# DeepMotionAIResearch/DenseMatchingBenchmark

Hardware: AMD Instinct MI355X
Metric: stereo pairs/s (540x960, max_disp=192) (higher is better)
Workload: dtype f32; 1 GPU; PSMNet Concatenation-volume + 3D aggregation + soft-argmin, 544x960 (540x960 padded), max_disp=192, batch 4 per GPU; costs_materialised=True, conv3d_mode=exact

## Files before the change

densematchingbenchmark_amd/csrc/catconv.hip:

```cpp
#include "dmb_common.h"

namespace dmb {

typedef float f32x4_t __attribute__((ext_vector_type(4)));

__global__ __launch_bounds__(256) void copy_window_kernel(const float* __restrict__ src, float* __restrict__ dst,
                                                          long long rows, int W, int Wd, int xs) {
  const long long total = rows * Wd;
  for (long long i = blockIdx.x * 256LL + threadIdx.x; i < total; i += (long long)gridDim.x * 256) {
    const long long r = i / Wd;
    const int j = (int)(i - r * Wd), g = j + xs;
    dst[i] = (g >= 0 && g < W) ? src[r * W + g] : 0.f;
  }
}

__global__ __launch_bounds__(256) void zero_columns_kernel(float* __restrict__ t, long long rows, int pitch, int x0) {
  const int n = pitch - x0;
  const long long total = rows * n;
  for (long long i = blockIdx.x * 256LL + threadIdx.x; i < total; i += (long long)gridDim.x * 256) {
    const long long r = i / n;
    t[r * pitch + x0 + (int)(i - r * n)] = 0.f;
  }
}

// ... 98 lines not shown
        f[e] = u >= 2 ? f[e] : (u >= -2 ? t : 0.f);
      }
    }
    const float g3 = border ? gbz : g[3];
    float4 o;
    o.x = fmaxf(fmaf(f[0] + g[0], sc, sh), lo);
    o.y = fmaxf(fmaf(f[1] + g[1], sc, sh), lo);
    o.z = fmaxf(fmaf(f[2] + g[2], sc, sh), lo);
    o.w = fmaxf(fmaf(f[3] + g3, sc, sh), lo);
    __builtin_nontemporal_store(f32x4_t{o.x, o.y, o.z, o.w}, reinterpret_cast<f32x4_t*>(op + (size_t)z * HW));
  };
  if (zlo == 0) {
    const float4 a1 = fa4(1), a2 = fa4(2);
    float g[4];
#pragma unroll
    for (int e = 0; e < 4; ++e) g[e] = hc1(1, x + e) + hc1(2, x + e - 1);
    plane(0, make_float4(a1.x + a2.x, a1.y + a2.y, a1.z + a2.z, a1.w + a2.w), g, band[0], gb[0]);
  }
  const float4 fm = *reinterpret_cast<const float4*>(FM + row * W + x);
  auto gml = [&](int n) { return gm_row[n > -4 ? n : -4]; };
  constexpr int ZB = 4;
  float win[ZB + 3], gbw[ZB];
  float4 bnd[ZB];
  auto load_block = [&](int z0, float (&w)[ZB + 3], float4 (&bq)[ZB], float (&gq)[ZB]) {
#pragma unroll
    for (int i = 0; i < ZB + 3; ++i) w[i] = gml(x - z0 + 3 - i);
#pragma unroll
    for (int k = 0; k < ZB; ++k) {
      const int z = z0 + k < D ? z0 + k : D - 1;
      if (NEAR) bq[k] = (x - z >= -5 && x - z <= 1) ? band[z] : make_float4(0.f, 0.f, 0.f, 0.f);
      if (!NEAR) gq[k] = gb[z];
    }
  };
  const int zb = zlo > 1 ? zlo : 1, ze = zhi < D - 1 ? zhi : D - 1;
  load_block(zb, win, bnd, gbw);
  for (int z0 = zb; z0 < ze; z0 += ZB) {
    float nwin[ZB + 3], ngbw[ZB];
    float4 nbnd[ZB];
    if (z0 + ZB < ze) load_block(z0 + ZB, nwin, nbnd, ngbw);
#pragma unroll
    for (int k = 0; k < ZB; ++k) {
      if (z0 + k < ze) {
        const float g[4] = {win[3 + k], win[2 + k], win[1 + k], win[k]};
        plane(z0 + k, fm, g, bnd[k], gbw[k]);
      }
    }
#pragma unroll
    for (int i = 0; i < ZB + 3; ++i) win[i] = nwin[i];
#pragma unroll
    for (int k = 0; k < ZB; ++k) {
      bnd[k] = nbnd[k];
      gbw[k] = ngbw[k];
    }
  }
  if (zhi == D) {
    const float4 a0 = fa4(0), a1 = fa4(1);
    const int u0 = x - (D - 1);
    float g[4];
#pragma unroll
    for (int e = 0; e < 4; ++e) g[e] = hc1(0, u0 + e + 1) + hc1(1, u0 + e);
    plane(D - 1, make_float4(a0.x + a1.x, a0.y + a1.y, a0.z + a1.z, a0.w + a1.w), g, band[D - 1], gb[D - 1]);
  }
}

template <bool NEAR>
__global__ __launch_bounds__(256) void catconv_combine_kernel(const float* __restrict__ FA, const float* __restrict__ HC,
                                                              const float* __restrict__ FM, const float* __restrict__ BAND,
                                                              const float* __restrict__ GM, const float* __restrict__ GB,
                                                              const float* __restrict__ scale, const float* __restrict__ shift,
                                                              float* __restrict__ out, long long rows, int Co, int CA, int D,
                                                              int H, int W, int XS, int relu) {
  constexpr int ZSPLIT = NEAR ? 4 : 1;
  const int W4 = NEAR ? XS >> 2 : (W - XS) >> 2;
  long long idx = blockIdx.x * 256LL + threadIdx.x;
  if (idx >= rows * W4 * ZSPLIT) return;
  const int zc = (int)(idx / (rows * W4));
  idx -= zc * (rows * W4);
  const long long rowid = idx / W4;
  const int dz = D / ZSPLIT;
  catconv_combine_body<NEAR>(FA, HC, FM, BAND, GM, GB, scale, shift, out, Co, CA, D, H, W, relu, rowid,
                             (int)(idx - rowid * W4) * 4 + (NEAR ? 0 : XS), zc * dz, (zc + 1) * dz);
}

}

using namespace dmb;

extern "C" int dmb_copy_window_f32(const float* src, float* dst, long long rows, int W, int Wd, int xs, void* stream) {
  if (!src || !dst || rows <= 0 || W <= 0 || Wd <= 0) return fail(DMB_EINVAL, "copy_window: bad argument");
  const long long total = rows * Wd;
  const int blocks = (int)((total + 255) / 256 < 65536 ? (total + 255) / 256 : 65536);
  hipLaunchKernelGGL(copy_window_kernel, dim3(blocks), dim3(256), 0, (hipStream_t)stream, src, dst, rows, W, Wd, xs);
  return launch_status("copy_window launch failed");
}

extern "C" int dmb_zero_columns_f32(float* t, long long rows, int pitch, int x0, void* stream) {
  if (!t || rows <= 0 || pitch <= 0 || x0 < 0 || x0 > pitch) return fail(DMB_EINVAL, "zero_columns: bad argument");
  if (x0 == pitch) return DMB_OK;
  const long long total = rows * (pitch - x0);
  const int blocks = (int)((total + 255) / 256 < 65536 ? (total + 255) / 256 : 65536);
  hipLaunchKernelGGL(zero_columns_kernel, dim3(blocks), dim3(256), 0, (hipStream_t)stream, t, rows, pitch, x0);
  return launch_status("zero_columns launch failed");
}

extern "C" int dmb_catconv_finalize_f32(const float* FA, const float* FB, const float* HC, const float* HD, float* FM,
                                        float* BAND, float* GM, float* GB, int B, int Co, int CA, int CB, int D, int H, int W,
                                        int Wc, void* stream) {
  if (!FA || !FB || !HC || !HD || !FM || !BAND || !GM || !GB || B <= 0 || Co <= 0 || D < 3 || H <= 0 || W <= 0 || (W & 3) ||
      CA < 3 * Co || CB < 6 * Co || (CB & 1) || Wc > W || Wc < D + 2 || (((uintptr_t)FA | (uintptr_t)FM) & 15))
    return fail(DMB_EINVAL, "catconv_finalize: bad argument");
  const long long rows = (long long)B * Co * H;
  if (rows > 0x7fffffffLL) return fail(DMB_EUNSUPPORTED, "catconv_finalize: grid too large");
  hipLaunchKernelGGL(catconv_finalize_kernel, dim3((unsigned)rows), dim3(256), 0, (hipStream_t)stream, FA, FB, HC, HD, FM, BAND,
                     GM, GB, B, Co, CA, CB, D, H, W, Wc);
  return launch_status("catconv_finalize launch failed");
}

extern "C" int dmb_catconv_combine_f32(const float* FA, const float* HC, const float* FM, const float* BAND, const float* GM,
                                       const float* GB, const float* scale, const float* shift, float* out, int B, int Co,
                                       int CA, int D, int H, int W, int relu, void* stream) {
  if (!FA || !HC || !FM || !BAND || !GM || !GB || !out || B <= 0 || Co <= 0 || CA < 3 * Co || D < 3 || (D & 3) || H <= 0 ||
      W <= 0 || (W & 3) || W < D + 8 || (((uintptr_t)FA | (uintptr_t)FM | (uintptr_t)BAND | (uintptr_t)out) & 15))
    return fail(DMB_EINVAL, "catconv_combine: bad argument (D, W multiples of 4, W >= D + 8, tensors 16-byte aligned)");
  int XS = (D + 4 + 15) / 16 * 16;
  if (XS > W - 4) XS = W - 4;
  const long long rows = (long long)B * Co * H, tn = rows * (XS / 4) * 4, tf = rows * ((W - XS) / 4);
  if ((tf + 255) / 256 > 0x7fffffffLL || (tn + 255) / 256 > 0x7fffffffLL) return fail(DMB_EUNSUPPORTED, "catconv_combine: grid too large");
  hipLaunchKernelGGL(catconv_combine_kernel<false>, dim3((unsigned)((tf + 255) / 256)), dim3(256), 0, (hipStream_t)stream, FA,
                     HC, FM, BAND, GM, GB, scale, shift, out, rows, Co, CA, D, H, W, XS, relu);
  hipLaunchKernelGGL(catconv_combine_kernel<true>, dim3((unsigned)((tn + 255) / 256)), dim3(256), 0, (hipStream_t)stream, FA,
                     HC, FM, BAND, GM, GB, scale, shift, out, rows, Co, CA, D, H, W, XS, relu);
  return launch_status("catconv_combine launch failed");
}
```

densematchingbenchmark_amd/ops.py:

```python
import ctypes

import torch

from . import _lib, param_state
from ._lib import check, dev_ptr, host_floats, host_ints, launch, opt, stream_ptr
from .param_state import bump_param_epoch, param_epoch


def disp_index_list(max_disp, start_disp=0, dilation=1):
    end_disp = start_disp + max_disp - 1
    n = (max_disp + dilation - 1) // dilation
    return [int(v) for v in torch.linspace(start_disp, end_disp, n)]


def disp_sample_values(max_disp, start_disp=0, dilation=1):
    end_disp = start_disp + max_disp - 1
    n = (max_disp + dilation - 1) // dilation
    return [float(v) for v in torch.linspace(start_disp, end_disp, n)]


class KernelTimer:

    def __init__(self, tags, every=1):
        self.tags = set(tags)
# ... 284 lines not shown
AUTO_OVERLAP_MAX_VOXELS = 48 * 136 * 240
_side_streams = {}


def set_branch_overlap(flag):
    global _branch_overlap
    _branch_overlap = "auto" if flag == "auto" else bool(flag)


def branch_overlap(raw_cost=None):
    if _branch_overlap != "auto":
        return _branch_overlap
    if raw_cost is None:
        return False
    B, _, D, H, W = raw_cost.shape
    return B * D * H * W <= AUTO_OVERLAP_MAX_VOXELS


def side_stream(device, which=0):
    key = (device.index if device.index is not None else torch.cuda.current_device(), which)
    if key not in _side_streams:
        _side_streams[key] = torch.cuda.Stream(device)
    return _side_streams[key]


_view_streams = True


def set_view_streams(flag):
    global _view_streams
    _view_streams = bool(flag)


def view_streams():
    return _view_streams


def warm_packed_parameters(module):
    stamp = param_state.module_stamp(module)
    if module.__dict__.get("_dmb_warmed") == stamp:
        return
    for m in module.modules():
        pre = getattr(m, "_prepacked", None)
        if pre is not None:
            pre()
    module.__dict__["_dmb_warmed"] = stamp


def _map_tensors(f, out):
    if torch.is_tensor(out):
        return f(out)
    return type(out)(_map_tensors(f, o) for o in out)


def two_view_forward(fn, left, right, module=None):
    if not (_view_streams and left.is_cuda):
        B = left.shape[0]
        f = fn(torch.cat((left, right), 0))
        return _map_tensors(lambda t: t[:B], f), _map_tensors(lambda t: t[B:], f)
    if module is not None:
        warm_packed_parameters(module)
    main = torch.cuda.current_stream(left.device)
    side = side_stream(left.device, 2)
    fork = main.record_event()
    with torch.cuda.stream(side):
        side.wait_event(fork)
        fr = fn(right)
        _map_tensors(lambda t: t.record_stream(main), fr)
        right.record_stream(side)
        done = side.record_event()
    fl = fn(left)
    main.wait_event(done)
    return fl, fr


_first_layer_mode = "merged"


def set_first_layer_mode(mode):
    global _first_layer_mode
    if mode not in ("merged", "streams", "serial"):
        raise ValueError("first-layer mode must be 'merged', 'streams' or 'serial'")
    _first_layer_mode = mode


def set_first_layer_streams(flag):
    set_first_layer_mode("streams" if flag else "serial")


def copy_window(src, Wd, xs):
    sh = _lib.shim()
    if sh is not None:
        return sh.copy_window(src if src.is_contiguous() else src.contiguous(), int(Wd), int(xs))
    src = _f32c(src, "src")
    W = src.shape[-1]
    dst = torch.empty(tuple(src.shape[:-1]) + (Wd,), dtype=torch.float32, device=src.device)
    launch("dmb_copy_window_f32", src, dst, src.numel() // W, W, Wd, xs)
    return dst


def zero_columns_(t, x0):
    if t.dtype != torch.float32 or not t.is_contiguous():
        raise _lib.DmbLibraryError("zero_columns_: contiguous float32 tensor expected")
    pitch = t.shape[-1]
    launch("dmb_zero_columns_f32", t, t.numel() // pitch, pitch, x0)
    return t


DECONV_PLAN_SPLIT_K, DECONV_PLAN_QUEUE, DECONV_PLAN_PARITY = 1, 2, 3
CONV_PLAN_SPLIT_K, CONV_PLAN_S1_VEC, CONV_PLAN_S1_FLAT, CONV_PLAN_S1_C128, CONV_PLAN_S2 = 1, 2, 3, 4, 5


def _align(t):
    p = 0 if t is None else t.data_ptr()
    return min(p & -p or 16, 16)


def conv3d_k3_plan(x, Co, stride=1, residual=None, out=None, ncu=0):
    shape = tuple(x) if isinstance(x, (tuple, list)) else tuple(x.shape)
    B, Ci, D, H, W = (int(v) for v in shape)
    xa = 16 if isinstance(x, (tuple, list)) else _align(x)
    stride = _hw_stride(stride, "conv3d_k3_plan")
    if stride == "hw":
        raise _lib.DmbLibraryError("conv3d_k3_plan: stride (1, 2, 2) is dmb_conv3d_k3_hw_f32's, which has one form")
    return _lib.load().dmb_conv3d_k3_plan(B, Ci, int(Co), D, H, W, int(stride), xa, _align(out), _align(residual), 0 if _split_k else 1, int(ncu))


def padded_rows_applicable(x, Co):
    B, Ci, D, H, W = x.shape
    if not (x.is_cuda and W % 4 == 2):
        return False
    plan = _lib.load().dmb_deconv3d_k3s2_plan(B, Ci, Co, D, H, (W + 3) // 4 * 4, 2 * W, min(x.data_ptr() & -x.data_ptr() or 16, 16), 16, 16, 16, 1, 0)
    return plan >> 8 == DECONV_PLAN_QUEUE


CATCONV_CH = 128


def catconv_applicable(L, R, disp_idx, Co):
    if not _cat_fusion or L.dim() != 4 or L.shape != R.shape:
        return False
    D, W = len(disp_idx), L.shape[3]
    return (list(disp_idx) == list(range(D)) and D >= 4 and D % 4 == 0 and W % 4 == 0 and W >= D + 8 and Co <= 32
            and L.dtype == torch.float32 and L.is_cuda)


def catconv_pack(w, kind="cat"):
    lib = _lib.load()
    w = _f32c(w.detach(), "weight")
    Co = w.shape[0]
    C = w.shape[1] if kind == "dif" else w.shape[1] // 2
    n = lib.dmb_conv2d_packed_floats(CATCONV_CH, C, 3)
    buf = torch.empty((5, n), dtype=torch.float32, device=w.device)
    launch("dmb_catconv_pack_weights_f32", w, buf, Co, C, CATCONV_CH, 1 if kind == "dif" else 0)
    return {"A": buf[0], "B1": buf[1], "B2": buf[2], "HC": buf[3], "HD": buf[4], "Co": Co, "Cin": C}


def catconv_pack_torch(w, kind="cat"):
    Co = w.shape[0]
    w = w.detach().float()
    if kind == "dif":
        wl, wr = w, -w
    else:
        C = w.shape[1] // 2
        wl, wr = w[:, :C], w[:, C:]
    C = wl.shape[1]

    def stack(half, dx_from, dx_to):
        k = torch.zeros((CATCONV_CH, C, 3, 3), dtype=torch.float32, device=w.device)
        for dz in range(3):
            k[dz * Co:(dz + 1) * Co, :, :, dx_from:dx_to] = half[:, :, dz, :, dx_from:dx_to]
        return pack_conv2d_weights(k)

    return {"A": stack(wl, 0, 3), "B1": stack(wl, 1, 3), "B2": stack(wl, 2, 3), "HC": stack(wr, 0, 3), "HD": stack(wr, 0, 2),
            "Co": Co, "Cin": C}


def catconv_first(L, R, D, packs, scale=None, shift=None, relu=False):
    L, R = _feature_pair(L, R, "catconv_first")
    B, C, H, W = L.shape
    if packs.get("Cin") is not None and packs["Cin"] != C:
        raise _lib.DmbLibraryError("catconv_first: weights were packed for %d feature channels, the maps have %d" % (packs["Cin"], C))
    Co, CA = packs["Co"], CATCONV_CH
    Wc = D + 4
    dev = L.device
    Lc, Rw, Rl = copy_window(L, Wc, 0), copy_window(R, W + 4, -4), copy_window(R, Wc, W - Wc)
    if _first_layer_mode == "merged":
        FA = torch.empty((B, CA, H, W), dtype=torch.float32, device=dev)
        HC = torch.empty((B, CA, H, W + 4), dtype=torch.float32, device=dev)
        FB = torch.empty((B, 2 * CA, H, Wc), dtype=torch.float32, device=dev)
        HD = torch.empty((B, CA, H, Wc), dtype=torch.float32, device=dev)
        conv2d_k3_multi([(Rw, packs["HC"], HC, 0), (L, packs["A"], FA, 0), (Lc, packs["B1"], FB, 0), (Lc, packs["B2"], FB, CA),
                         (Rl, packs["HD"], HD, 0)], CA)
    elif _first_layer_mode == "streams":
        main = torch.cuda.current_stream(dev)
        s1, s2 = side_stream(dev), side_stream(dev, 1)
        fork = main.record_event()
        with torch.cuda.stream(s1):
            s1.wait_event(fork)
            FB = torch.empty((B, 2 * CA, H, Wc), dtype=torch.float32, device=dev)
            conv2d(Lc, packs["B1"], CA, 3, out=FB, out_ch_offset=0)
            conv2d(Lc, packs["B2"], CA, 3, out=FB, out_ch_offset=CA)
            FB.record_stream(main)
            j1 = s1.record_event()
        with torch.cuda.stream(s2):
            s2.wait_event(fork)
            HD = conv2d(Rl, packs["HD"], CA, 3)
            HD.record_stream(main)
            j2 = s2.record_event()
        FA, HC = conv2d(L, packs["A"], CA, 3), conv2d(Rw, packs["HC"], CA, 3)
        main.wait_event(j1)
        main.wait_event(j2)
    else:
        FA, HC = conv2d(L, packs["A"], CA, 3), conv2d(Rw, packs["HC"], CA, 3)
        FB = torch.empty((B, 2 * CA, H, Wc), dtype=torch.float32, device=dev)
        conv2d(Lc, packs["B1"], CA, 3, out=FB, out_ch_offset=0)
        conv2d(Lc, packs["B2"], CA, 3, out=FB, out_ch_offset=CA)
        HD = conv2d(Rl, packs["HD"], CA, 3)
    FM = torch.empty((B, Co, H, W), dtype=torch.float32, device=dev)
    BAND = torch.empty((B, Co, H, D, 4), dtype=torch.float32, device=dev)
    GM = torch.empty((B, Co, H, W + 4), dtype=torch.float32, device=dev)
    GB = torch.empty((B, Co, H, D), dtype=torch.float32, device=dev)
    launch("dmb_catconv_finalize_f32", FA, FB, HC, HD, FM, BAND, GM, GB, B, Co, CA, 2 * CA, D, H, W, Wc)
    out = torch.empty((B, Co, D, H, W), dtype=torch.float32, device=dev)
    launch("dmb_catconv_combine_f32", FA, HC, FM, BAND, GM, GB, opt(scale), opt(shift), out, B, Co, CA, D, H, W, _relu_mode(relu))
    return out


_conv3d_mode = "exact"


def set_conv3d_mode(mode):
    global _conv3d_mode
    if mode not in ("exact", "bf16x6"):
        raise ValueError("conv3d mode must be 'exact' or 'bf16x6'")
    _conv3d_mode = mode


def conv3d_mode():
    return _conv3d_mode


def conv3d_x6_applicable(x, Co, stride):
    W = x.shape[-1]
    return stride == 1 and ((Co == 32 and W % 48 == 0) or (Co == 64 and W % 24 == 0)) and x.data_ptr() % 16 == 0


def pack_conv3d_x6_weights(w):
    lib = _lib.load()
    w = _f32c(w, "weight")
    Co, Ci = w.shape[0], w.shape[1]
    wp = torch.empty((lib.dmb_conv3d_x6_packed_bytes(Co, Ci) // 4,), dtype=torch.float32, device=w.device)
    launch("dmb_conv3d_x6_pack_weights_f32", w, wp, Co, Ci)
    return wp


def conv3d_k3_x6(x, wpack, Co, scale=None, shift=None, residual=None, relu=False):
    lib = _lib.load()
    B, Ci, D, H, W = x.shape
    return _unit_conv3d(lib.dmb_conv3d_k3_x6_f32, "conv3d_k3_s1_%dto%d" % (Ci, Co), "conv3d_k3_x6", x, wpack, scale, shift, residual,
                        None, (B, Co, D, H, W), lib.dmb_conv3d_x6_packed_bytes(Co, Ci) // 4, (B, Ci, Co, D, H, W), (_relu_mode(relu),))


def conv3d_k3_c1(x, w, bias=0.0, residual=None):
    sh = _lib.shim()
    if sh is not None:
        return sh.conv3d_k3_c1(x if x.is_contiguous() else x.contiguous(), w if w.is_contiguous() else w.contiguous(), float(bias),
                               residual, _conv_flags())
    x, w = _f32c(x, "x"), _f32c(w, "weight")
    B, Ci, D, H, W = x.shape
    y = torch.empty((B, 1, D, H, W), dtype=torch.float32, device=x.device)
    if w.numel() != Ci * 27:
        raise _lib.DmbLibraryError("conv3d_k3_c1: weight %s for %d input channels" % (tuple(w.shape), Ci))
    if residual is not None:
        _same_shape(residual, y, "conv3d_k3_c1 residual")
    launch("dmb_conv3d_k3_c1_f32", x, w, bias, opt(residual), y, B, Ci, D, H, W, _conv_flags())
    return y


_deconv_ws = {}


def deconv3d_workspace(device):
    if torch.cuda.is_current_stream_capturing():
        return torch.zeros((_lib.DECONV3D_WORKSPACE_BYTES // 4,), dtype=torch.int32, device=device)
    st = torch.cuda.current_stream(device)
    key = (device.index if device.index is not None else torch.cuda.current_device(), st.cuda_stream)
    ws = _deconv_ws.get(key)
    if ws is None:
        ws = torch.zeros((_lib.DECONV3D_WORKSPACE_BYTES // 4,), dtype=torch.int32, device=device)
        _deconv_ws[key] = ws
    return ws


def deconv3d_k3s2(x, wpack, Co, scale=None, shift=None, residual=None, relu=False, workspace="auto", out=None, out_width=None,
                  stride=(2, 2, 2)):
    stride = tuple(int(s) for s in stride) if isinstance(stride, (tuple, list)) else (int(stride),) * 3
    if stride == (1, 2, 2):
        if not (isinstance(workspace, str) and workspace == "auto") or out_width is not None:
            raise _lib.DmbLibraryError("deconv3d_k3s2: stride (1, 2, 2) takes no workspace and no out_width")
        lib = _lib.load()
        B, Ci, D, H, W = x.shape
        return _unit_conv3d(lib.dmb_deconv3d_k3_hw_f32, "deconv3d_k3_s122_%dto%d" % (Ci, Co), "deconv3d_k3s2", x, wpack, scale, shift,
                            residual, out, (B, Co, D, 2 * H, 2 * W), lib.dmb_deconv3d_packed_floats(Ci, Co), (B, Ci, Co, D, H, W),
                            (_relu_mode(relu) | _conv_flags(),))
    if stride != (2, 2, 2):
        raise _lib.DmbLibraryError("deconv3d_k3s2: stride %s is not built: (2, 2, 2) or (1, 2, 2)" % (stride,))
    sh = _lib.shim()
# ... 1111 lines not shown
```

include/dmb_hip.h:

```cpp
#ifndef DMB_HIP_H
#define DMB_HIP_H

#ifdef __cplusplus
extern "C" {
#endif

#define DMB_OK 0
#define DMB_EINVAL 100001
#define DMB_EUNSUPPORTED 100002

#define DMB_MAX_DISP_SAMPLES 256

#define DMB_ABI_VERSION 13
int dmb_abi_version(void);
const char* dmb_last_error(void);
const char* dmb_build_id(void);


int dmb_cat_fms_f32(const float* L, const float* R, float* out, int B, int C, int H, int W, int D,
                    const int* disp_idx_host, void* stream);

int dmb_dif_fms_f32(const float* L, const float* R, float* out, int B, int C, int H, int W, int D,
                    const int* disp_idx_host, void* stream);

int dmb_fast_cat_fms_f32(const float* L, const float* R, const float* disp_sample, float* out, int B, int C, int D, int H,
                         int W, int per_pixel, void* stream);

int dmb_fast_dif_fms_f32(const float* L, const float* R, const float* disp_sample, float* out, int B, int C, int D, int H,
                         int W, int per_pixel, int normalize, float p, void* stream);

int dmb_fast_fms_bwd_f32(const float* L, const float* R, const float* disp_sample, const float* dvol, const float* norm_out,
                         float* dL, float* dR, float* d_samples, float* partial, int B, int C, int D, int H, int W,
                         int per_pixel, int mode, float p, void* stream);

int dmb_spn_gaterecurrent2d_f32(const float* X, const float* G1, const float* G2, const float* G3, float* H_out, int N, int C,
                                int H, int W, int horizontal, int reverse, void* stream);
int dmb_spn_gaterecurrent2d_bwd_f32(const float* X, const float* G1, const float* G2, const float* G3, const float* H_fwd,
                                    const float* dH, float* dX, float* dG1, float* dG2, float* dG3, int N, int C, int H, int W,
                                    int horizontal, int reverse, void* stream);

int dmb_gwc_fms_f32(const float* L, const float* R, float* out, int B, int C, int G, int H, int W, int D,
                    const int* disp_idx_host, int out_channels, int out_ch_offset, void* stream);

int dmb_catconv_pack_weights_f32(const float* w, float* packs, int Co, int C, int CA, int dif, void* stream);
int dmb_copy_window_f32(const float* src, float* dst, long long rows, int W, int Wd, int xs, void* stream);
int dmb_zero_columns_f32(float* t, long long rows, int pitch, int x0, void* stream);
int dmb_catconv_finalize_f32(const float* FA, const float* FB, const float* HC, const float* HD, float* FM, float* BAND,
                             float* GM, float* GB, int B, int Co, int CA, int CB, int D, int H, int W, int Wc, void* stream);
int dmb_catconv_combine_f32(const float* FA, const float* HC, const float* FM, const float* BAND, const float* GM,
                            const float* GB, const float* scale, const float* shift, float* out, int B, int Co, int CA, int D,
                            int H, int W, int relu, void* stream);

int dmb_correlation1d_f32(const float* L, const float* R, float* out, int B, int C, int H, int W, int D,
                          float negative_slope, void* stream);

int dmb_cat_fms_into_f32(const float* L, const float* R, float* out, int B, int C, int H, int W, int D,
                         const int* disp_idx_host, int out_channels, int out_ch_offset, void* stream);

#define DMB_CONV_SINGLE_CHAIN 0x100

long long dmb_conv3d_packed_floats(int Co, int Ci);
long long dmb_deconv3d_packed_floats(int Ci, int Co);

int dmb_conv3d_pack_weights_f32(const float* w, float* wpack, int Co, int Ci, void* stream);
int dmb_deconv3d_pack_weights_f32(const float* w, float* wpack, int Ci, int Co, void* stream);

int dmb_conv3d_k3_f32(const float* x, const float* wpack, const float* scale, const float* shift,
                      const float* residual, float* y, int B, int Ci, int Co, int D, int H, int W,
                      int stride, int relu, void* stream);
int dmb_conv3d_k3_plan(int B, int Ci, int Co, int D, int H, int W, int stride, int x_align, int y_align, int residual_align,
                       int single_chain, int ncu);

int dmb_conv3d_k3_c1_f32(const float* x, const float* w, float bias, const float* residual, float* y,
                         int B, int Ci, int D, int H, int W, int flags, void* stream);

#define DMB_CONV3D_HEAD_PACKED_FLOATS 1024
long long dmb_conv3d_k3_head_workspace_floats(int B, int D, int H, int W);
int dmb_conv3d_k3_head_preferred(int B, int D, int H, int W);
int dmb_conv3d_head_pack_weights_f32(const float* w_head, float* head_wpack, void* stream);
int dmb_conv3d_k3_head_f32(const float* x, const float* wpack, const float* scale, const float* shift,
                           const float* head_wpack, float bias, const float* residual, float* y, float* workspace,
                           int B, int Ci, int D, int H, int W, int relu, void* stream);
int dmb_conv3d_k3_head_partial_f32(const float* x, const float* wpack, const float* scale, const float* shift,
                                   const float* head_wpack, float* workspace, int B, int Ci, int D, int H, int W, int relu,
                                   void* stream);
int dmb_conv3d_head_chain_finish_f32(int nlevels, const float* const* workspaces, const float* bias_host, const float* residual,
                                     float* const* y, int B, int D, int H, int W, void* stream);

#define DMB_DECONV3D_WORKSPACE_BYTES 2048
int dmb_deconv3d_k3s2_f32(const float* x, const float* wpack, const float* scale, const float* shift,
                          const float* residual, float* y, int B, int Ci, int Co, int D, int H, int W, int Wout,
                          int relu, void* workspace, void* stream);
int dmb_deconv3d_k3s2_plan(int B, int Ci, int Co, int D, int H, int W, int Wout, int x_align, int y_align, int residual_align,
                           int workspace_align, int single_chain, int ncu);

int dmb_conv3d_k3_hw_f32(const float* x, const float* wpack, const float* scale, const float* shift,
                         const float* residual, float* y, int B, int Ci, int Co, int D, int H, int W,
                         int stride_hw, int relu, void* stream);

int dmb_deconv3d_k3_hw_f32(const float* x, const float* wpack, const float* scale, const float* shift,
                           const float* residual, float* y, int B, int Ci, int Co, int D, int H, int W, int relu,
                           void* stream);


int dmb_trilinear_ac_f32(const float* x, float* y, int B, int Di, int Hi, int Wi, int Do, int Ho, int Wo,
                         void* stream);

int dmb_deconv3d_k8s4_c1_f32(const float* x, const float* w, float* y, int B, int D, int H, int W,
                             void* stream);

int dmb_deconv3d_k8s4_c1_soft_argmin_f32(const float* x, const float* w, float* y, float* disp, int B, int D, int H, int W,
                                         float alpha, const float* disp_sample_host, void* stream);


int dmb_soft_argmin_f32(const float* cost, float* disp, int B, int D, int H, int W, float alpha,
                        int normalize, const float* disp_sample_host, void* stream);

int dmb_soft_argmin_sampled_f32(const float* cost, const float* sample, float* disp, int B, int D, int H,
                                int W, float alpha, int normalize, void* stream);

int dmb_local_soft_argmin_f32(const float* cost, float* disp, long long* argidx, int B, int D, int H, int W,
                              int radius, int radius_dilation, int start_disp, int dilation, float alpha,
                              void* stream);

int dmb_trilinear_ac_soft_argmin_f32(const float* x, float* y, float* disp, int B, int Di, int Hi, int Wi, int Do,
                                     int Ho, int Wo, float alpha, const float* disp_sample_host, void* stream);

int dmb_trilinear_soft_argmin_f32(const float* x, float* disp, int B, int Di, int Hi, int Wi, int Do, int Ho,
                                  int Wo, float alpha, const float* disp_sample_host, void* stream);

#define DMB_UPSAMPLE_TRILINEAR_AC 1
// ... 243 lines not shown
```

Measured before the change: 152.0 pairs/s.

## Fuse catconv finalize and combine into a single one-pass kernel

Adds a one-pass combine kernel for the first-layer concatenation conv. It reads the FA/FB/HC/HD partial products directly and rebuilds the FM, BAND, GM and GB terms on the fly in registers with a sliding window, instead of materialising those intermediates in a separate finalize kernel. The far and near column regions now share one launch, using a block-index split, and the inner loops use vectorised float4 loads. This removes a kernel launch and the intermediate tensor traffic, at the cost of more per-thread arithmetic and register pressure, and more complex boundary logic.

```diff
diff --git a/densematchingbenchmark_amd/csrc/catconv.hip b/densematchingbenchmark_amd/csrc/catconv.hip
--- a/densematchingbenchmark_amd/csrc/catconv.hip
+++ b/densematchingbenchmark_amd/csrc/catconv.hip
@@ -204,6 +204,375 @@
                              (int)(idx - rowid * W4) * 4 + (NEAR ? 0 : XS), zc * dz, (zc + 1) * dz);
 }
 
+template <bool NEAR>
+__device__ __forceinline__ void catconv_onepass_body(const float* __restrict__ FA, const float* __restrict__ FB,
+                                                     const float* __restrict__ HC, const float* __restrict__ HD,
+                                                     const float* __restrict__ scale, const float* __restrict__ shift,
+                                                     float* __restrict__ out, int Co, int CA, int CB, int D, int H, int W, int relu,
+                                                     long long rowid, int x, int zlo, int zhi) {
+  const int Wg = W + 4, Wc = D + 4;
+  long long r = rowid;
+  const int y = (int)(r % H); r /= H;
+  const int co = (int)(r % Co);
+  const int b = (int)(r / Co);
+  const float sc = scale ? scale[co] : 1.f, sh = shift ? shift[co] : 0.f;
+  const float lo = relu ? 0.f : -__builtin_inff();
+  const size_t HW = (size_t)H * W;
+  float* op = out + (((size_t)b * Co + co) * D) * HW + (size_t)y * W + x;
+  const bool border = !NEAR && x + 4 == W;
+  const float* hc[3];
+  const float* hd[3];
+  float A[3][4], B1[3][4], B2[3][4];
+  const bool banded = NEAR && x <= D && x + 5 >= zlo && x - 1 < zhi;
+#pragma unroll
+  for (int dz = 0; dz < 3; ++dz) {
+    const size_t mr = ((size_t)b * CA + dz * Co + co) * H + y;
+    hc[dz] = HC + mr * Wg + 4;
+    hd[dz] = HD + mr * Wc;
+    const float4 a = *reinterpret_cast<const float4*>(FA + mr * W + x);
+    A[dz][0] = a.x; A[dz][1] = a.y; A[dz][2] = a.z; A[dz][3] = a.w;
+    float4 p = make_float4(0.f, 0.f, 0.f, 0.f), q = p;
+    if (banded) {
+      p = *reinterpret_cast<const float4*>(FB + (((size_t)b * CB + dz * Co + co) * H + y) * Wc + x);
+      q = *reinterpret_cast<const float4*>(FB + (((size_t)b * CB + CB / 2 + dz * Co + co) * H + y) * Wc + x);
+    }
+    B1[dz][0] = p.x; B1[dz][1] = p.y; B1[dz][2] = p.z; B1[dz][3] = p.w;
+    B2[dz][0] = q.x; B2[dz][1] = q.y; B2[dz][2] = q.z; B2[dz][3] = q.w;
+  }
+  auto hc1 = [&](int dz, int n) { return n >= -4 ? hc[dz][n] : 0.f; };
+  auto gcol = [&](int n) {
+    const int nn = n > -4 ? n : -4;
+    float s = 0.f;
+    s += hc[0][nn + 1];
+    s += hc[1][nn];
+    const float c = hc[2][nn > -4 ? nn - 1 : -4];
+    return nn > -4 ? s + c : s;
+  };
+  auto gbv = [&](int z) {
+    const int v = z == 0 ? 0 : (z == D - 1 ? 2 : 1);
+    float s = 0.f;
+#pragma unroll
+    for (int dz = 0; dz < 3; ++dz) {
+      const int jj = Wc - z - dz;
+      if (z_tap_valid(v, dz) && jj >= 0 && jj < Wc) s += hd[dz][jj];
+    }
+    return s;
+  };
+  auto plane = [&](int z, const float (&fv)[4], const float (&g)[4], float gbz) {
+    float f[4] = {fv[0], fv[1], fv[2], fv[3]};
+    if (NEAR) {
+      if (x - z >= -5 && x - z <= 1) {
+        const int v = z == 0 ? 0 : (z == D - 1 ? 2 : 1);
+#pragma unroll
+        for (int e = 0; e < 4; ++e) {
+          const int u = x + e - z;
+          float s = 0.f;
+#pragma unroll
+          for (int dz = 0; dz < 3; ++dz) {
+            const int m = dz - u > 0 ? dz - u : 0;
+            const float a0 = A[dz][e], a1 = B1[dz][e], a2 = B2[dz][e];
+            const float t = m == 0 ? +a0 : (m == 1 ? +a1 : +a2);
+            s = (z_tap_valid(v, dz) && m <= 2) ? s + t : s;
+          }
+          f[e] = u >= 2 ? f[e] : (u >= -2 ? s : 0.f);
+        }
+      } else {
+#pragma unroll
+        for (int e = 0; e < 4; ++e) f[e] = x + e - z >= 2 ? f[e] : 0.f;
+      }
+    }
+    const float g3 = border ? gbz : g[3];
+    float4 o;
+    o.x = fmaxf(fmaf(f[0] + g[0], sc, sh), lo);
+    o.y = fmaxf(fmaf(f[1] + g[1], sc, sh), lo);
+    o.z = fmaxf(fmaf(f[2] + g[2], sc, sh), lo);
+    o.w = fmaxf(fmaf(f[3] + g3, sc, sh), lo);
+    __builtin_nontemporal_store(f32x4_t{o.x, o.y, o.z, o.w}, reinterpret_cast<f32x4_t*>(op + (size_t)z * HW));
+  };
+  if (zlo == 0) {
+    float f[4], g[4];
+#pragma unroll
+    for (int e = 0; e < 4; ++e) {
+      f[e] = A[1][e] + A[2][e];
+      g[e] = hc1(1, x + e) + hc1(2, x + e - 1);
+    }
+    plane(0, f, g, border ? gbv(0) : 0.f);
+  }
+  float fm[4];
+#pragma unroll
+  for (int e = 0; e < 4; ++e) fm[e] = A[0][e] + A[1][e] + A[2][e];
+  constexpr int ZB = 4;
+  float win[ZB + 3], gbw[ZB];
+  const int zb = zlo > 1 ? zlo : 1, ze = zhi < D - 1 ? zhi : D - 1;
+  auto load_gb = [&](int z0, float (&gq)[ZB]) {
+#pragma unroll
+    for (int k = 0; k < ZB; ++k) gq[k] = border ? gbv(z0 + k < D ? z0 + k : D - 1) : 0.f;
+  };
+#pragma unroll
+  for (int i = 0; i < ZB + 3; ++i) win[i] = gcol(x - zb + 3 - i);
+  load_gb(zb, gbw);
+  for (int z0 = zb; z0 < ze; z0 += ZB) {
+    float nwin[ZB + 3], ngbw[ZB];
+#pragma unroll
+    for (int i = 0; i < 3; ++i) nwin[i] = win[i + ZB];
+    if (z0 + ZB < ze) {
+#pragma unroll
+      for (int i = 3; i < ZB + 3; ++i) nwin[i] = gcol(x - (z0 + ZB) + 3 - i);
+      load_gb(z0 + ZB, ngbw);
+    }
+#pragma unroll
+    for (int k = 0; k < ZB; ++k) {
+      if (z0 + k < ze) {
+        const float g[4] = {win[3 + k], win[2 + k], win[1 + k], win[k]};
+        plane(z0 + k, fm, g, gbw[k]);
+      }
+    }
+#pragma unroll
+    for (int i = 0; i < ZB + 3; ++i) win[i] = nwin[i];
+#pragma unroll
+    for (int k = 0; k < ZB; ++k) gbw[k] = ngbw[k];
+  }
+  if (zhi == D) {
+    const int u0 = x - (D - 1);
+    float f[4], g[4];
+#pragma unroll
+    for (int e = 0; e < 4; ++e) {
+      f[e] = A[0][e] + A[1][e];
+      g[e] = hc1(0, u0 + e + 1) + hc1(1, u0 + e);
+    }
+    plane(D - 1, f, g, border ? gbv(D - 1) : 0.f);
+  }
+}
+
+template <bool NEAR>
+__device__ __forceinline__ void catconv_onepass_vec(const float* __restrict__ FA, const float* __restrict__ FB,
+                                                    const float* __restrict__ HC, const float* __restrict__ HD,
+                                                    const float* __restrict__ scale, const float* __restrict__ shift,
+                                                    float* __restrict__ out, int Co, int CA, int CB, int D, int H, int W, int relu,
+                                                    long long rowid, int x, int zlo, int zhi) {
+  constexpr int ZB = 4;
+  const int Wg = W + 4, Wc = D + 4;
+  long long r = rowid;
+  const int y = (int)(r % H); r /= H;
+  const int co = (int)(r % Co);
+  const int b = (int)(r / Co);
+  const float sc = scale ? scale[co] : 1.f, sh = shift ? shift[co] : 0.f;
+  const float lo = relu ? 0.f : -__builtin_inff();
+  const size_t HW = (size_t)H * W;
+  float* op = out + (((size_t)b * Co + co) * D) * HW + (size_t)y * W + x;
+  const bool border = !NEAR && x + 4 == W;
+  const float* hc[3];
+  const float* hd[3];
+  float A[3][4], B1[3][4], B2[3][4];
+  const bool banded = NEAR && x <= D && x + 5 >= zlo && x - 1 < zhi;
+#pragma unroll
+  for (int dz = 0; dz < 3; ++dz) {
+    const size_t mr = ((size_t)b * CA + dz * Co + co) * H + y;
+    hc[dz] = HC + mr * Wg + 4;
+    hd[dz] = HD + mr * Wc;
+    const float4 a = *reinterpret_cast<const float4*>(FA + mr * W + x);
+    A[dz][0] = a.x; A[dz][1] = a.y; A[dz][2] = a.z; A[dz][3] = a.w;
+    float4 p = make_float4(0.f, 0.f, 0.f, 0.f), q = p;
+    if (banded) {
+      p = *reinterpret_cast<const float4*>(FB + (((size_t)b * CB + dz * Co + co) * H + y) * Wc + x);
+      q = *reinterpret_cast<const float4*>(FB + (((size_t)b * CB + CB / 2 + dz * Co + co) * H + y) * Wc + x);
+    }
+    B1[dz][0] = p.x; B1[dz][1] = p.y; B1[dz][2] = p.z; B1[dz][3] = p.w;
+    B2[dz][0] = q.x; B2[dz][1] = q.y; B2[dz][2] = q.z; B2[dz][3] = q.w;
+  }
+  auto quad = [](const float* p, float (&v)[4]) {
+    const float4 t = *reinterpret_cast<const float4*>(p);
+    v[0] = t.x; v[1] = t.y; v[2] = t.z; v[3] = t.w;
+  };
+  auto hquad = [&](int dz, int n, float (&v)[4]) {
+    if (!NEAR || n >= -4) {
+      quad(hc[dz] + n, v);
+    } else {
+      v[0] = v[1] = v[2] = v[3] = 0.f;
+    }
+  };
+  auto hc1 = [&](int dz, int n) { return n >= -4 ? hc[dz][n] : 0.f; };
+  float gm4 = 0.f;
+  if (NEAR) {
+    gm4 += hc[0][-3];
+    gm4 += hc[1][-4];
+  }
+  auto gbv = [&](int z) {
+    const int v = z == 0 ? 0 : (z == D - 1 ? 2 : 1);
+    float s = 0.f;
+#pragma unroll
+    for (int dz = 0; dz < 3; ++dz) {
+      const int jj = Wc - z - dz;
+      if (z_tap_valid(v, dz) && jj >= 0 && jj < Wc) s += hd[dz][jj];
+    }
+    return s;
+  };
+  auto load_gb = [&](int z0, float (&gq)[ZB]) {
+    if (border) {
+      const int q = Wc - z0 - 3;
+      float d0[4], d1[8], d2[8];
+      quad(hd[0] + q, d0);
+      quad(hd[1] + q - 4, reinterpret_cast<float (&)[4]>(d1[0]));
+      quad(hd[1] + q, reinterpret_cast<float (&)[4]>(d1[4]));
+      quad(hd[2] + q - 4, reinterpret_cast<float (&)[4]>(d2[0]));
+      quad(hd[2] + q, reinterpret_cast<float (&)[4]>(d2[4]));
+#pragma unroll
+      for (int k = 0; k < ZB; ++k) {
+        float s = 0.f;
+        s += d0[3 - k];
+        s += d1[6 - k];
+        s += d2[5 - k];
+        gq[k] = s;
+      }
+    } else {
+#pragma unroll
+      for (int k = 0; k < ZB; ++k) gq[k] = 0.f;
+    }
+  };
+  auto store = [&](int z, const float (&fv)[4], const float (&g)[4], float gbz) {
+    float f[4] = {fv[0], fv[1], fv[2], fv[3]};
+    if (NEAR) {
+      if (x - z >= -5 && x - z <= 1) {
+        const int v = z == 0 ? 0 : (z == D - 1 ? 2 : 1);
+#pragma unroll
+        for (int e = 0; e < 4; ++e) {
+          const int u = x + e - z;
+          float s = 0.f;
+#pragma unroll
+          for (int dz = 0; dz < 3; ++dz) {
+            const int m = dz - u > 0 ? dz - u : 0;
+            const float a0 = A[dz][e], a1 = B1[dz][e], a2 = B2[dz][e];
+            const float t = m == 0 ? +a0 : (m == 1 ? +a1 : +a2);
+            s = (z_tap_valid(v, dz) && m <= 2) ? s + t : s;
+          }
+          f[e] = u >= 2 ? f[e] : (u >= -2 ? s : 0.f);
+        }
+      } else {
+#pragma unroll
+        for (int e = 0; e < 4; ++e) f[e] = x + e - z >= 2 ? f[e] : 0.f;
+      }
+    }
+    const float g3 = border ? gbz : g[3];
+    float4 o;
+    o.x = fmaxf(fmaf(f[0] + g[0], sc, sh), lo);
+    o.y = fmaxf(fmaf(f[1] + g[1], sc, sh), lo);
+    o.z = fmaxf(fmaf(f[2] + g[2], sc, sh), lo);
+    o.w = fmaxf(fmaf(f[3] + g3, sc, sh), lo);
+    __builtin_nontemporal_store(f32x4_t{o.x, o.y, o.z, o.w}, reinterpret_cast<f32x4_t*>(op + (size_t)z * HW));
+  };
+  const int zb = zlo > 1 ? zlo : 1, ze = zhi < D - 1 ? zhi : D - 1;
+  const int n0 = x - zb - 3;
+  float h0[8], h1[8], h2[12];
+  hquad(0, n0, reinterpret_cast<float (&)[4]>(h0[0]));
+  hquad(0, n0 + 4, reinterpret_cast<float (&)[4]>(h0[4]));
+  hquad(1, n0, reinterpret_cast<float (&)[4]>(h1[0]));
+  hquad(1, n0 + 4, reinterpret_cast<float (&)[4]>(h1[4]));
+  hquad(2, n0 - 4, reinterpret_cast<float (&)[4]>(h2[0]));
+  hquad(2, n0, reinterpret_cast<float (&)[4]>(h2[4]));
+  hquad(2, n0 + 4, reinterpret_cast<float (&)[4]>(h2[8]));
+  float win[ZB + 3], gbw[ZB];
+#pragma unroll
+  for (int i = 0; i < ZB + 3; ++i) {
+    float s = 0.f;
+    s += h0[7 - i];
+    s += h1[6 - i];
+    s += h2[9 - i];
+    win[i] = (NEAR && n0 + 6 - i <= -4) ? gm4 : s;
+  }
+  float c0 = h0[0];
+  float c2[4] = {h2[0], h2[1], h2[2], h2[3]};
+  if (zlo == 0) {
+    float f[4], g[4];
+#pragma unroll
+    for (int e = 0; e < 4; ++e) {
+      f[e] = A[1][e] + A[2][e];
+      g[e] = h1[4 + e] + h2[7 + e];
+    }
+    const float gb0 = border ? gbv(0) : 0.f;
+    load_gb(1, gbw);
+    store(0, f, g, gb0);
+  } else {
+    load_gb(zb, gbw);
+  }
+  float fm[4];
+#pragma unroll
+  for (int e = 0; e < 4; ++e) fm[e] = A[0][e] + A[1][e] + A[2][e];
+  for (int z0 = zb; z0 < ze; z0 += ZB) {
+    float nwin[ZB + 3], ngbw[ZB];
+#pragma unroll
+    for (int i = 0; i < 3; ++i) nwin[i] = win[i + ZB];
+    if (z0 + ZB < ze) {
+      const int n = x - (z0 + ZB) - 3;
+      float a0[4], a1[4], a2[4];
+      hquad(0, n, a0);
+      hquad(1, n, a1);
+      hquad(2, n - 4, a2);
+#pragma unroll
+      for (int k = 0; k < ZB; ++k) {
+        float s = 0.f;
+        s += k < 3 ? a0[k < 3 ? k + 1 : 0] : c0;
+        s += a1[k];
+        s += k == 0 ? a2[3] : c2[k > 0 ? k - 1 : 0];
+        nwin[6 - k] = (NEAR && n + k <= -4) ? gm4 : s;
+      }
+      c0 = a0[0];
+#pragma unroll
+      for (int k = 0; k < 4; ++k) c2[k] = a2[k];
+      load_gb(z0 + ZB, ngbw);
+    }
+#pragma unroll
+    for (int k = 0; k < ZB; ++k) {
+      if (z0 + k < ze) {
+        const float g[4] = {win[3 + k], win[2 + k], win[1 + k], win[k]};
+        store(z0 + k, fm, g, gbw[k]);
+      }
+    }
+#pragma unroll
+    for (int i = 0; i < ZB + 3; ++i) win[i] = nwin[i];
+#pragma unroll
+    for (int k = 0; k < ZB; ++k) gbw[k] = ngbw[k];
+  }
+  if (zhi == D) {
+    const int u0 = x - (D - 1);
+    float f[4], g[4];
+#pragma unroll
+    for (int e = 0; e < 4; ++e) {
+      f[e] = A[0][e] + A[1][e];
+      g[e] = hc1(0, u0 + e + 1) + hc1(1, u0 + e);
+    }
+    store(D - 1, f, g, border ? gbv(D - 1) : 0.f);
+  }
+}
+
+__global__ __launch_bounds__(256) void catconv_onepass_kernel(const float* __restrict__ FA, const float* __restrict__ FB,
+                                                              const float* __restrict__ HC, const float* __restrict__ HD,
+                                                              const float* __restrict__ scale, const float* __restrict__ shift,
+                                                              float* __restrict__ out, long long rows, int Co, int CA, int CB,
+                                                              int D, int H, int W, int XS, int relu, unsigned far_blocks) {
+  if (blockIdx.x < far_blocks) {
+    const int W4 = (W - XS) >> 2;
+    const long long idx = blockIdx.x * 256LL + threadIdx.x;
+    if (idx >= rows * W4) return;
+    const long long rowid = idx / W4;
+    catconv_onepass_vec<false>(FA, FB, HC, HD, scale, shift, out, Co, CA, CB, D, H, W, relu, rowid, (int)(idx - rowid * W4) * 4 + XS,
+                               0, D);
+  } else {
+    const int W4 = XS >> 2;
+    long long idx = (blockIdx.x - far_blocks) * 256LL + threadIdx.x;
+    if (idx >= rows * W4 * 4) return;
+    const int zc = (int)(idx / (rows * W4));
+    idx -= zc * (rows * W4);
+    const long long rowid = idx / W4;
+    const int dz = D / 4, xq = (int)(idx - rowid * W4) * 4;
+    if ((dz & 3) == 0) {
+      catconv_onepass_vec<true>(FA, FB, HC, HD, scale, shift, out, Co, CA, CB, D, H, W, relu, rowid, xq, zc ? 1 + zc * dz : 0,
+                                zc == 3 ? D : 1 + (zc + 1) * dz);
+    } else {
+      catconv_onepass_body<true>(FA, FB, HC, HD, scale, shift, out, Co, CA, CB, D, H, W, relu, rowid, xq, zc * dz, (zc + 1) * dz);
+    }
+  }
+}
+
 }
 
 using namespace dmb;
@@ -238,9 +607,26 @@
   return launch_status("catconv_finalize launch failed");
 }
 
+static int catconv_onepass(const float* FA, const float* FB, const float* HC, const float* HD, const float* scale, const float* shift,
+                           float* out, int B, int Co, int CA, int CB, int D, int H, int W, int relu, void* stream) {
+  if (!FA || !FB || !HC || !HD || !out || B <= 0 || Co <= 0 || CA < 3 * Co || CB < 6 * Co || (CB & 1) || D < 3 || (D & 3) ||
+      H <= 0 || W <= 0 || (W & 3) || W < D + 8 || (((uintptr_t)FA | (uintptr_t)FB | (uintptr_t)HC | (uintptr_t)HD | (uintptr_t)out) & 15))
+    return fail(DMB_EINVAL, "catconv_combine (one pass): bad argument (D, W multiples of 4, W >= D + 8, tensors 16-byte aligned)");
+  int XS = (D + 4 + 15) / 16 * 16;
+  if (XS > W - 4) XS = W - 4;
+  const long long rows = (long long)B * Co * H, tn = rows * (XS / 4) * 4, tf = rows * ((W - XS) / 4);
+  const long long bf = (tf + 255) / 256, bn = (tn + 255) / 256;
+  if (bf + bn > 0x7fffffffLL) return fail(DMB_EUNSUPPORTED, "catconv_combine (one pass): grid too large");
+  hipLaunchKernelGGL(catconv_onepass_kernel, dim3((unsigned)(bf + bn)), dim3(256), 0, (hipStream_t)stream, FA, FB, HC, HD, scale,
+                     shift, out, rows, Co, CA, CB, D, H, W, XS, relu, (unsigned)bf);
+  return launch_status("catconv_combine (one pass) launch failed");
+}
+
 extern "C" int dmb_catconv_combine_f32(const float* FA, const float* HC, const float* FM, const float* BAND, const float* GM,
                                        const float* GB, const float* scale, const float* shift, float* out, int B, int Co,
                                        int CA, int D, int H, int W, int relu, void* stream) {
+  if (relu & DMB_CATCONV_ONE_PASS)
+    return catconv_onepass(FA, FM, HC, BAND, scale, shift, out, B, Co, CA, 2 * CA, D, H, W, relu & ~DMB_CATCONV_ONE_PASS, stream);
   if (!FA || !HC || !FM || !BAND || !GM || !GB || !out || B <= 0 || Co <= 0 || CA < 3 * Co || D < 3 || (D & 3) || H <= 0 ||
       W <= 0 || (W & 3) || W < D + 8 || (((uintptr_t)FA | (uintptr_t)FM | (uintptr_t)BAND | (uintptr_t)out) & 15))
     return fail(DMB_EINVAL, "catconv_combine: bad argument (D, W multiples of 4, W >= D + 8, tensors 16-byte aligned)");
diff --git a/densematchingbenchmark_amd/ops.py b/densematchingbenchmark_amd/ops.py
--- a/densematchingbenchmark_amd/ops.py
+++ b/densematchingbenchmark_amd/ops.py
@@ -390,6 +390,16 @@
     if mode not in ("merged", "streams", "serial"):
         raise ValueError("first-layer mode must be 'merged', 'streams' or 'serial'")
     _first_layer_mode = mode
+
+
+_first_layer_combine = "one_pass"
+
+
+def set_first_layer_combine(form):
+    global _first_layer_combine
+    if form not in ("one_pass", "two_pass"):
+        raise ValueError("first-layer combine must be 'one_pass' or 'two_pass'")
+    _first_layer_combine = form
 
 
 def set_first_layer_streams(flag):
@@ -525,13 +535,17 @@
         conv2d(Lc, packs["B1"], CA, 3, out=FB, out_ch_offset=0)
         conv2d(Lc, packs["B2"], CA, 3, out=FB, out_ch_offset=CA)
         HD = conv2d(Rl, packs["HD"], CA, 3)
-    FM = torch.empty((B, Co, H, W), dtype=torch.float32, device=dev)
-    BAND = torch.empty((B, Co, H, D, 4), dtype=torch.float32, device=dev)
-    GM = torch.empty((B, Co, H, W + 4), dtype=torch.float32, device=dev)
-    GB = torch.empty((B, Co, H, D), dtype=torch.float32, device=dev)
-    launch("dmb_catconv_finalize_f32", FA, FB, HC, HD, FM, BAND, GM, GB, B, Co, CA, 2 * CA, D, H, W, Wc)
     out = torch.empty((B, Co, D, H, W), dtype=torch.float32, device=dev)
-    launch("dmb_catconv_combine_f32", FA, HC, FM, BAND, GM, GB, opt(scale), opt(shift), out, B, Co, CA, D, H, W, _relu_mode(relu))
+    if _first_layer_combine == "two_pass":
+        FM = torch.empty((B, Co, H, W), dtype=torch.float32, device=dev)
+        BAND = torch.empty((B, Co, H, D, 4), dtype=torch.float32, device=dev)
+        GM = torch.empty((B, Co, H, W + 4), dtype=torch.float32, device=dev)
+        GB = torch.empty((B, Co, H, D), dtype=torch.float32, device=dev)
+        launch("dmb_catconv_finalize_f32", FA, FB, HC, HD, FM, BAND, GM, GB, B, Co, CA, 2 * CA, D, H, W, Wc)
+        launch("dmb_catconv_combine_f32", FA, HC, FM, BAND, GM, GB, opt(scale), opt(shift), out, B, Co, CA, D, H, W, _relu_mode(relu))
+    else:
+        launch("dmb_catconv_combine_f32", FA, HC, FB, HD, opt(None), opt(None), opt(scale), opt(shift), out, B, Co, CA, D, H, W,
+               _relu_mode(relu) | _lib.DEFINES["DMB_CATCONV_ONE_PASS"])
     return out
 
 
diff --git a/include/dmb_hip.h b/include/dmb_hip.h
--- a/include/dmb_hip.h
+++ b/include/dmb_hip.h
@@ -47,6 +47,7 @@
 int dmb_zero_columns_f32(float* t, long long rows, int pitch, int x0, void* stream);
 int dmb_catconv_finalize_f32(const float* FA, const float* FB, const float* HC, const float* HD, float* FM, float* BAND,
                              float* GM, float* GB, int B, int Co, int CA, int CB, int D, int H, int W, int Wc, void* stream);
+#define DMB_CATCONV_ONE_PASS 0x100
 int dmb_catconv_combine_f32(const float* FA, const float* HC, const float* FM, const float* BAND, const float* GM,
                             const float* GB, const float* scale, const float* shift, float* out, int B, int Co, int CA, int D,
                             int H, int W, int relu, void* stream);
```

Result: no change. 152.3 pairs/s, median of 6 (+0.2%).
